# Griffan/FASTQuick

Measured on AMD Instinct MI355X. Metric: paired_150bp_reads_aligned_per_sec, higher is better.
Workload: dtype u32

## Files before the change

fastquick_amd/csrc/fq_align.cpp:

```cpp
#include <algorithm>
#include <atomic>
#include <ctime>
#include <chrono>
#include <climits>
#include <cstdint>
#include <cmath>
#include <cstdio>
#include <cstdlib>
#include <cstring>
#include <memory>
#include <string>
#include <unordered_map>
#include <mutex>
#include <thread>
#include <vector>
#include <pthread.h>
#include <sched.h>

#include "../../include/fastquick_amd.h"
#include "fq_backend.h"
#include "fq_index.h"
#include "fq_pipeline.h"
#include "fq_pool.h"
#include "fq_text_batch.h"
// ... 128 lines not shown
    }
    used = 0; total = 0; last_grow = tl_grow;
  }
  void *alloc(size_t bytes) {
    bytes = (bytes + 63) & ~(size_t)63;
    total += bytes;
    if (blocks.empty() || used + bytes > blocks.back().cap) {
      size_t cap = std::max<size_t>(std::max(bytes, grown(bytes)), (size_t)4 << 20);
      uint8_t *p = (uint8_t *)obtain(cap, true, &cap);
      if (!p) return nullptr;
      blocks.push_back({p, cap});
      used = 0;
    }
    void *r = blocks.back().p + used;
    used += bytes;
    return r;
  }
};

struct FqKnobs {
  uint32_t gap_long_pops = 256;
  int gap_long_always = 0;
  int64_t gap_skip_bound = -1;
  uint32_t gap_long_pops2 = 0;
  int64_t gap_split_hard = 0;
  int64_t gap_pipeline_min = -1;
  int gap_pipeline_segs = 8;
  int64_t gap_nogap_min = 131072;
  uint32_t gap_pool = 2048;
  int gap_no_order = 0;
  int device_turns = 2;
  int device_turn_slots = 1;
  int64_t device_turn_min = 1 << 20;
  int gap_round2_refill = 16;
  int gap_round1_refill = 0;
  int gap_round2_lane_major = 1;
  int gap_round2_waves = 2560;
  int sw_wave_max = 4096;
  int host_threads = -1;
  size_t host_par_min = 32768;
  int64_t md_mask_min = 4096;
  int64_t packed_bulk_min = -1;
  int trace = 0;
};

struct SearchBufs {
  DevBuf<int32_t> work;
  DevBuf<uint32_t> wfull; DevBuf<FqPos> prec; DevBuf<FqGapWork> winfo; DevBuf<uint8_t> bid_end;
  DevBuf<int32_t> order; DevBuf<uint32_t> order_cnt;
  DevBuf<FqAln> aln; DevBuf<uint32_t> naln, status;
  DevBuf<uint32_t> queue, heads; DevBuf<FqEntry> pool;
};

struct fq_ctx {
  FqWorkPool pool;
  const fq_index *ix = nullptr;
  fq_opts_t o{};
  FqKOpts ko{};
  FqKnobs kn;
  fqdev::State *dev = nullptr;
  int max_pairs = 0;
  int debug = 0;
  std::string err;
  fq_serial_hook before_serial = nullptr, after_serial = nullptr;
  void *hook_user = nullptr;
  bool serial_open = false, serial_done = false;
  bool stream_broken = false;
  uint64_t rng = 0;
  fq_isize_t last_ii{};
  std::unordered_map<uint64_t, vector<uint32_t>> kl_cache;
  int g_log_n[256];
  uint8_t maxdiff_lut[FQ_LMAX + 2];
  int n_pairs = 0, stride = 0;
  int in_kind = 0;
  fq_read_batch_t hb{};
  fq_packed_batch_t pb{};
  const fq_text_batch *tb = nullptr;
  PinBuf<uint8_t> p_cseq, p_cqual;
  PinBuf<int32_t> p_clen;
  PinBuf<char> p_cnames;
  DevBuf<char> d_cnames;
  vector<uint16_t> h_len_all;
  int c_stride = 0, c_name_stride = 0;
  DevBuf<uint64_t> d_head[2];
  DevBuf<uint16_t> d_hlen[2];
  DevBuf<uint8_t> d_qlast[2];
  int head_slot = 0;
  const fq_packed_batch_t *pend[2] = {nullptr, nullptr};
  uint64_t pend_serial[2] = {0, 0};
  bool is_pending(int i, const fq_packed_batch_t *b) const { return pend[i] == b && pend_serial[i] == b->serial; }
  DevBuf<uint8_t> d_body, d_pqual;
  DevBuf<uint64_t> d_exc;
  DevBuf<int32_t> d_row_map, d_crow, d_len_c, d_len_all;
  PinBuf<uint8_t> p_body, p_pqual;
  PinBuf<uint64_t> p_exc;
  PinBuf<uint16_t> p_hlen;
  DevBuf<uint16_t> d_blen;
  DevBuf<uint8_t> d_seq, d_qual, d_filtered, d_maxdiff;
  DevBuf<int32_t> d_len, d_len_trim, d_read_list, d_sidx, d_pair_list, d_counts;
  DevBuf<uint64_t> d_counters;
  std::vector<uint64_t> h_counters;
  SearchBufs sb[2];
  DevBuf<uint32_t> d_seg_cnt;
  DevBuf<FqAln> d_hits;
  DevBuf<uint64_t> d_aoff; DevBuf<uint32_t> d_an;
  DevBuf<uint64_t> d_off;
  DevBuf<FqDRec> d_rec, d_grec;
  DevBuf<uint32_t> d_nocc, d_qfirst, d_cnt[3], d_isz;
  DevBuf<uint16_t> d_ntop;
  DevBuf<uint8_t> d_enum, d_cls;
  DevBuf<uint64_t> d_row0, d_scan[3], d_rng, d_grow0;
  DevBuf<int32_t> d_list, d_refmax;
  DevBuf<fq_multi_t> d_multi, d_omulti;
  DevBuf<FqSwTask> d_swslot; DevBuf<FqSwCand> d_swcand;
  DevBuf<FqPairRead> d_greads; DevBuf<FqPairOut> d_gout;
  DevBuf<FqRefTgt> d_reftgt;
  DevBuf<uint16_t> d_cigs, d_ocig;
  DevBuf<fq_isize_t> d_iis;
  DevBuf<fq_result_t> d_orec;
  DevBuf<char> d_omd;
  PinBuf<fq_result_t> p_orec; PinBuf<uint16_t> p_ocig; PinBuf<char> p_omd; PinBuf<fq_multi_t> p_omulti;
  PinBuf<uint16_t> p_ntop; PinBuf<uint32_t> p_isz; PinBuf<int32_t> p_pairs;
  DevBuf<FqAln> d_qaln;
  DevBuf<uint32_t> d_qlen, d_pos, d_qpos, d_qrow, d_qinfo;
  DevBuf<FqPairIsize> d_pisize; DevBuf<int32_t> d_plut, d_glogn; DevBuf<uint64_t> d_pscratch;
  DevBuf<uint64_t> d_qoff;
  DevBuf<FqSwTask> d_swtask;
  DevBuf<FqSwOut> d_swout;
  DevBuf<FqRefTask> d_reftask;
  DevBuf<FqRefOut> d_refout;
  DevBuf<uint16_t> d_cig, d_cigarena;
  DevBuf<uint8_t> d_scratch;
  DevBuf<char> d_md;
  DevBuf<uint16_t> d_mdmask;
  vector<uint8_t> h_filtered;
  vector<int32_t> h_len_trim, h_sub_max;
  const int32_t *h_pair_list = nullptr;
  const FqSurvInfo *h_surv = nullptr;
  Retired retired;
  PinArena arena;
  PinBuf<int32_t> p_i32;
  PinBuf<FqSurvInfo> p_surv;
  PinBuf<uint32_t> p_u32a, p_u32b, p_pos;
  PinBuf<FqAln> p_aln;
  DevBuf<FqSurvInfo> d_surv;
  DevBuf<int32_t> d_sub_max;
  int64_t n_bases_in = 0;
  int emit_flags = 0;
  bool host_rows = true;
  DevBuf<uint8_t> d_equal; PinBuf<uint8_t> p_equal;
  DevBuf<char> d_enames; PinBuf<char> p_enames;
  int e_qstride = 0, e_nstride = 0;
  std::mutex view_mu;
  bool view_ready = false;
  FqSamArgs view{};
  vector<uint8_t> h_eseq;
  DevBuf<uint32_t> d_samlen, d_sammeta; DevBuf<uint64_t> d_samoff; DevBuf<char> d_samtext;
  uint64_t sam_bytes = 0;
  bool sam_ready = false;
  fqdev::State *dev_emit[2] = {nullptr, nullptr};
  PinBuf<char> p_emit[2][2];
  fq_bam *bam = nullptr;
  DevBuf<uint32_t> d_bamlen, d_bammeta, d_zsize; DevBuf<uint64_t> d_bamoff, d_zoff; DevBuf<uint8_t> d_bamrec, d_zstage, d_bamz;
  FqBamCallOut bam_out;
  PinBuf<uint64_t> p_ztotal;
  uint32_t emit_nb = 0;
  std::mutex emit_mu;
  bool emit_pending = false;
  fq_qc *qc = nullptr;
  DevBuf<int32_t> d_qadded;
  DevBuf<uint32_t> d_istlen, d_ptcnt;
  DevBuf<uint64_t> d_istoff, d_ptoff, d_qcnt, d_dupkey;
  DevBuf<char> d_isttext; DevBuf<FqPileEntry> d_pile;
// ... 1721 lines not shown
      c->stats.d2h_bytes += N * sizeof(fq_result_t) + cc * 2 + mm + xx * sizeof(fq_multi_t);
    }
  }
  uint64_t cnt[FQ_C_COUNT];
  c->h_counters.resize((size_t)FQ_C_STRIPES * FQ_C_STRIDE);
  CKS(d2h_staged(c, c->h_counters.data(), c->d_counters.p, c->h_counters.size() * 8));
  CKS(sync_staged(c));
  fold_counters(c->h_counters.data(), cnt);
  CK(fqdev::dzero(c->d_counters.p, c->h_counters.size() * 8));
  if (!N && ((c->emit_flags & FQ_EMIT_SAM) || c->qc || c->bam)) CKS(emit_measure(K));
  if (host_arrays) {
    if (!cc) c->p_ocig.p[0] = 0;
    if (!mm) c->p_omd.p[0] = 0;
    if (!xx) c->p_omulti.p[0] = fq_multi_t{};
  }
  K.trace("result arrays D2H");
  if (cnt[FQ_C_ERR_DRAW0]) {
    c->err = "the drand48 stream drew exactly 0 for the first best hit of a read (once in 2^48 draws): bwa_aln2seq_core then takes no hit and the reference's "
             "record keeps the SA row of the read slot's previous occupant (libbwa/bwase.c:29-41) -- its result is undefined, and so this call is refused";
    return FQ_ELIMIT;
  }
  if (cnt[FQ_C_ERR_CIGAR]) { c->err = "refine: CIGAR longer than the device slot"; return FQ_ELIMIT; }
  if (cnt[FQ_C_ERR_MD]) { c->err = "MD string longer than the device slot"; return FQ_ELIMIT; }
  if (host_arrays) { S.rec = c->p_orec.p; S.cigar = c->p_ocig.p; S.md = c->p_omd.p; S.multi = c->p_omulti.p; }
  else { S.rec = nullptr; S.cigar = nullptr; S.md = nullptr; S.multi = nullptr; }
  S.n_both_unmapped = (int)cnt[FQ_C_UNMAPPED];
  out->n_survivors = n_surv;
  out->n_both_filtered = K.n - n_surv;
  out->n_both_unmapped = S.n_both_unmapped;
  out->pair_idx = S.pair_idx;
  out->rec = S.rec;
  out->cigar = S.cigar;
  out->md = S.md;
  out->multi = S.multi;
  out->isize = K.iis[n_sub - 1];
  out->n_sub = n_sub;
  out->isize_sub = S.isize_sub.data();
  out->n_bases = c->n_bases_in;
  fqdev::time_collect(c->stats.kernel_ms, c->stats.kernel_launches, FQ_K_COUNT);
  c->stats.occ_block_touches += cnt[FQ_C_OCC_WIDTH] + cnt[FQ_C_OCC_GAP] + cnt[FQ_C_OCC_SA];
  c->stats.gap_occ_touches += cnt[FQ_C_OCC_GAP];
  c->stats.width_occ_touches += cnt[FQ_C_OCC_WIDTH];
  c->stats.md_reads += cnt[FQ_C_MD_READS];
  c->stats.host_pairs += (uint64_t)K.n_host_pairs;
  c->stats.gap_nogap_touches += cnt[FQ_C_OCC_NOGAP];
  c->stats.filter_probes += cnt[FQ_C_PROBES];
  c->stats.stack_pops += cnt[FQ_C_POPS];
  c->stats.stack_pushes += cnt[FQ_C_PUSHES];
  if (cnt[FQ_C_MAXPOPS] > c->stats.max_pops_per_read) c->stats.max_pops_per_read = cnt[FQ_C_MAXPOPS];
  c->stats.reads_over_4k_pops += cnt[FQ_C_POPS_GT4K];
  if (cnt[FQ_C_MAXTRIPS] > c->stats.max_wave_trips) c->stats.max_wave_trips = cnt[FQ_C_MAXTRIPS];
  c->stats.wave_trips += cnt[FQ_C_SUMTRIPS];
  c->stats.lane_trips += cnt[FQ_C_LANETRIPS];
  c->stats.sa_rows += cnt[FQ_C_SA_DIRECT];
  c->stats.pairs_on_device += cnt[FQ_C_PAIRS_DEV];
  for (int k = 0; k < 16; ++k) c->stats.dbg[k] += cnt[FQ_C_DBG0 + k];
  c->stats.pairs += K.n;
  c->stats.host_ms_serial += (K.t_serial1 - K.t_host0) - (K.w_serial1 - K.w_host0);
  c->stats.host_ms_pair += (K.t_host1 - K.t_serial1) - (K.w_host1 - K.w_serial1);
  c->stats.host_ms_total += (K.t_host1 - K.t_host0) - (K.w_host1 - K.w_host0);
  c->stats.wall_ms_total += now_ms() - K.t_wall0;
  c->stats.device_wait_ms += c->wait_ms - K.w_call0;
  { timespec ts; clock_gettime(CLOCK_THREAD_CPUTIME_ID, &ts); c->stats.host_cpu_ms += 1e3 * (double)ts.tv_sec + 1e-6 * (double)ts.tv_nsec - K.cpu_call0; }
  K.trace("counters+timers");
  if ((c->emit_flags & FQ_EMIT_SAM) || c->qc || c->bam) CKS(emit_fill(K));
  return FQ_OK;
}
#undef REC

int run_call_stages(fq_ctx *c, fq_result_batch_t *out);
int run_call(fq_ctx *c, fq_result_batch_t *out) {
  c->serial_open = c->serial_done = false;
  const int rc = run_call_stages(c, out);
  if (rc && (c->before_serial || c->after_serial)) {
    c->stream_broken = true;
    if (!c->serial_open && !c->serial_done && c->before_serial) c->before_serial(c->hook_user);
    if (!c->serial_done && c->after_serial) c->after_serial(c->hook_user);
  }
  if (rc) {
    fqdev::copy_discard();
    (void)fqdev::stream_aux(0);
    (void)fqdev::dzero(c->d_counters.p, (size_t)FQ_C_STRIPES * FQ_C_STRIDE * 8);
    (void)fqdev::sync();
    (void)fqdev::copy_wait(0);
    (void)fqdev::copy_wait(1);
  }
  return rc;
}
int run_call_stages(fq_ctx *c, fq_result_batch_t *out) {
  CallInFlight in_flight(c->ix);
  Call K(c);
  K.t_trace = K.t_wall0 = now_ms();
  K.w_call0 = c->wait_ms;
  { timespec ts; clock_gettime(CLOCK_THREAD_CPUTIME_ID, &ts); K.cpu_call0 = 1e3 * (double)ts.tv_sec + 1e-6 * (double)ts.tv_nsec; }
  NodePin pin;
  struct PoolScope { FqWorkPool *prev; explicit PoolScope(FqWorkPool *p) : prev(tl_pool) { tl_pool = p; } ~PoolScope() { tl_pool = prev; } } pool_scope(&c->pool);
  (void)fqdev::stream_aux(0);
  const double grow = c->in_kind == 3 && c->tb && c->n_pairs > 0 && std::min<double>((double)c->max_pairs, (double)c->tb->pairs_behind) > (double)c->n_pairs
                          ? std::min(16.0, std::min<double>((double)c->max_pairs, (double)c->tb->pairs_behind) / (double)c->n_pairs) : 1.0;
  GrowScope grow_scope(grow);
  c->retired.next_call();
  RetiredScope retired_scope(&c->retired);
  if (c->kn.trace) { fprintf(stderr, "[fq]   arena: %zu blocks, last call used %zu bytes:", c->arena.blocks.size(), c->arena.total); for (auto &b : c->arena.blocks) fprintf(stderr, " %zu", b.cap); fprintf(stderr, "\n"); }
  c->arena.reset();
  const fq_opts_t &o = c->o;
  FqBatchState &S = c->st;
  S.clear();
  S.n_pairs = c->n_pairs;
  c->e_qstride = c->e_nstride = 0; c->view_ready = false;
  memset(out, 0, sizeof *out);
  out->n_pairs = c->n_pairs;
  if (c->n_pairs == 0) {
    const int rc0 = emit_measure(K);
    return rc0 ? rc0 : emit_fill(K);
  }
  K.n = c->n_pairs; K.n2 = 2 * K.n; K.B = o.batch_pairs; K.n_sub = (K.n + K.B - 1) / K.B;
  K.par_min = c->kn.host_par_min;
  K.host_threads = call_host_threads(c);
  int rc = c->in_kind == 3 ? stage0_text(K) : c->in_kind == 2 ? stage0_packed(K) : stage0_ascii(K);
  if (rc) return rc;
  S.n_surv = K.n_surv;
  S.batch_pairs = K.B;
  S.sub_lo = K.sub_lo;
  S.pair_idx = c->h_pair_list;
  S.surv = c->h_surv;
  K.trace("stage0 prep+compact");
  if ((rc = stageA_search(K))) return rc;
  K.trace("stageA width+gap");
  if ((rc = stage_records(K))) return rc;
  K.trace("records, SA plan, best-hit counts D2H");
  K.plan.n_chunks = ((size_t)K.n_surv + FQ_RNG_CHUNK_PAIRS - 1) / FQ_RNG_CHUNK_PAIRS;
  K.plan.start = (uint64_t *)c->arena.alloc((K.plan.n_chunks + 1) * 8);
  if (!K.plan.start) { c->err = "out of pinned host memory"; return FQ_ENOMEM; }
  if (!c->before_serial && (size_t)K.n_surv * 2 >= K.par_min) K.plan_thread = std::thread([&K, c] { stageB1_plan(K, c->rng); });
  if ((rc = stage_sa_rows(K))) return rc;
  K.trace("SA enumerate+kernel");
  K.t_host0 = now_ms(); K.w_host0 = c->wait_ms;
  if (c->before_serial) c->before_serial(c->hook_user);
  c->serial_open = true;
  if (c->stream_broken) { c->err = "the stream's state comes from a call that failed (on this rank or on the one before)"; return FQ_EIO; }
  if ((rc = stageB1_main_hit(K))) return rc;
  K.trace("B1 replay + main hit");
  if (o.single_end) K.iis.assign(K.n_sub, fq_isize_t{});
  else {
    stageB2_isize(K);
    c->last_ii = K.iis[K.n_sub - 1];
    if ((rc = stage_kl_cache(K))) return rc;
  }
  K.gate_take(c->qc);
  if (c->after_serial) c->after_serial(c->hook_user);
  c->serial_done = true;
  if (c->stream_broken) { c->err = "the hook that hands the stream's state on failed (fq_ctx_mark_stream_broken)"; return FQ_EIO; }
  K.t_serial1 = now_ms(); K.w_serial1 = c->wait_ms;
  K.trace("B2 isize, (k,l) cache");
  if ((rc = stageB3_pairing(K))) return rc;
  K.trace("B3 pairing+XA");
  if (c->debug && (rc = snapshot_records(K, S.stage_P))) return rc;
  if (!o.single_end && (rc = stageC_mate_sw(K))) return rc;
  K.trace("C mate SW");
  if (c->debug && (rc = snapshot_records(K, S.stage_S))) return rc;
  if ((rc = stageD_refine(K))) return rc;
  K.trace("D refine+MD");
  K.t_host1 = now_ms(); K.w_host1 = c->wait_ms;
  return stage_finish(K, out);
}
}

extern "C" int fq_host_cpus(void) { return (int)effective_cpus(); }
extern "C" int fq_runtime_configure(int hw_queues, int blocking_waits) { return fqdev::runtime_configure(hw_queues, blocking_waits); }
extern "C" int fq_device_count(void) { return fqdev::device_count(); }

extern "C" int fq_align_resident(fq_ctx_t *c, fq_result_batch_t *out) {
  if (!c || !out) return FQ_EINVAL;
  if (c->in_kind != 1) { c->err = "fq_align_resident: no batch uploaded (fq_batch_upload)"; return FQ_EINVAL; }
  if (fqdev::bind(c->dev)) return FQ_ENODEV;
  return run_call(c, out);
}

static int packed_check(fq_ctx_t *c, const fq_packed_batch_t *in) {
  if (!in || in->n_pairs < 0 || (in->n_pairs > 0 && (!in->head || !in->body || in->body_stride < 1 || (in->uniform_len <= 0 && !in->len)))) return FQ_EINVAL;
  if (in->n_exc < 0 || (in->n_exc > 0 && !in->exc)) return FQ_EINVAL;
  if (in->n_pairs > c->max_pairs) { c->err = "batch larger than max_pairs_per_batch"; return FQ_ELIMIT; }
  if (in->uniform_len > 0 && (in->uniform_len < FQ_LMIN || in->uniform_len > FQ_LMAX || (in->uniform_len + 3) / 4 > in->body_stride)) return refuse_length(c);
  if (c->o.trim_qual >= 1 && in->n_pairs > 0 && (!in->qual || in->qual_stride < 1)) { c->err = "quality trimming needs the batch's qualities"; return FQ_EINVAL; }
  if (in->n_pairs > 0 && in->qual_last && !in->qual) { c->err = "qual_last without the quality rows"; return FQ_EINVAL; }
  if ((in->single_end != 0) != (c->o.single_end != 0)) { c->err = c->o.single_end ? "a single-end context takes single-end batches (fq_pack_single_reads_into)" : "a paired-end context takes paired batches"; return FQ_EINVAL; }
  return FQ_OK;
}
extern "C" int fq_packed_prefetch(fq_ctx_t *c, const fq_packed_batch_t *next) {
  if (!c) return FQ_EINVAL;
  int rc = packed_check(c, next);
  if (rc) return rc;
  if (fqdev::bind(c->dev)) return FQ_ENODEV;
  if (next->n_pairs == 0 || c->is_pending(0, next) || c->is_pending(1, next)) return FQ_OK;
  for (int i = 0; i < 2; ++i) if (c->pend[i] == next) c->pend[i] = nullptr;
  const int slot = !c->pend[0] ? 0 : !c->pend[1] ? 1 : -1;
  if (slot < 0) return FQ_OK;
  rc = head_upload(c, next, slot);
  if (rc) return rc;
  c->pend[slot] = next; c->pend_serial[slot] = next->serial;
  return FQ_OK;
}
extern "C" int fq_packed_cancel(fq_ctx_t *c, const fq_packed_batch_t *b) {
  if (!c || !b) return FQ_EINVAL;
  for (int i = 0; i < 2; ++i)
    if (c->pend[i] == b) {
      if (fqdev::bind(c->dev)) return FQ_ENODEV;
      CK(fqdev::copy_wait(i));
      c->pend[i] = nullptr;
    }
  return FQ_OK;
}
extern "C" int fq_align_packed(fq_ctx_t *c, const fq_packed_batch_t *in, fq_result_batch_t *out) {
  if (!c || !out) return FQ_EINVAL;
  int rc = packed_check(c, in);
  if (rc) return broken_stream_call(c, rc);
  if (fqdev::bind(c->dev)) return FQ_ENODEV;
  c->pb = *in;
  c->n_pairs = in->n_pairs;
  c->in_kind = 2;
  if (in->n_pairs > 0) {
    if (c->is_pending(0, in)) { c->head_slot = 0; c->pend[0] = nullptr; }
    else if (c->is_pending(1, in)) { c->head_slot = 1; c->pend[1] = nullptr; }
    else {
      for (int i = 0; i < 2; ++i) if (c->pend[i] == in) c->pend[i] = nullptr;
      c->head_slot = !c->pend[0] ? 0 : 1;
      c->pend[c->head_slot] = nullptr;
      rc = head_upload(c, in, c->head_slot);
      if (rc) return broken_stream_call(c, rc);
    }
  }
  return run_call(c, out);
}

extern "C" int fq_stream_run(fq_ctx_t *const *ctxs, int32_t n_streams, const fq_packed_batch_t *const *const *batches, const int32_t *n_batches, const int32_t *first,
                             int32_t n_calls, int32_t flags, fq_stream_call_fn on_call, void *user, int64_t *survivors_out) {
  if (!ctxs || n_streams < 1 || !batches || !n_batches || n_calls < 0) return FQ_EINVAL;
  for (int s = 0; s < n_streams; ++s) if (!ctxs[s] || !batches[s] || n_batches[s] < 1) return FQ_EINVAL;
  for (int s = 0; s < n_streams; ++s) for (int t = 0; t < s; ++t) if (ctxs[s] == ctxs[t]) return FQ_EINVAL;
  std::vector<int> rcs((size_t)n_streams, FQ_OK);
  std::vector<int64_t> surv((size_t)n_streams, 0);
  static const bool trace_cpu = [] { const char *e = getenv("FASTQUICK_TRACE"); return e && *e && *e != '0'; }();
  std::vector<double> cpu_pre((size_t)n_streams, 0.0), cpu_call((size_t)n_streams, 0.0);
  auto thread_cpu_ms = [] { timespec ts; clock_gettime(CLOCK_THREAD_CPUTIME_ID, &ts); return 1e3 * (double)ts.tv_sec + 1e-6 * (double)ts.tv_nsec; };
  auto run = [&](int s) {
    fq_ctx_t *c = ctxs[s];
    const int nb = n_batches[s];
    int cur = (first ? first[s] : 0) % nb;
    if (cur < 0) cur += nb;
    fq_result_batch_t res;
    for (int k = 0; k < n_calls; ++k) {
      const int nxt = (cur + 1) % nb;
      int rc = FQ_OK;
      const bool pre = nxt != cur && (k + 1 < n_calls || (flags & FQ_STREAM_PREFETCH_BEYOND));
      const double c0 = trace_cpu ? thread_cpu_ms() : 0.0;
      if (pre) rc = fq_packed_prefetch(c, batches[s][nxt]);
      const double c1 = trace_cpu ? thread_cpu_ms() : 0.0;
      if (!rc) rc = fq_align_packed(c, batches[s][cur], &res);
      if (trace_cpu) { cpu_pre[(size_t)s] += c1 - c0; cpu_call[(size_t)s] += thread_cpu_ms() - c1; }
      if (!rc) { surv[(size_t)s] += res.n_survivors; if (on_call) rc = on_call(user, s, k, &res); }
      if (rc) { rcs[(size_t)s] = rc; if (pre) (void)fq_packed_cancel(c, batches[s][nxt]); return; }
      cur = nxt;
    }
  };
  std::vector<std::thread> th;
  for (int s = 1; s < n_streams; ++s) th.emplace_back(run, s);
  run(0);
  for (auto &t : th) t.join();
  if (survivors_out) for (int s = 0; s < n_streams; ++s) survivors_out[s] = surv[(size_t)s];
  if (trace_cpu && n_calls > 0) {
    double a = 0, b = 0;
    for (int s = 0; s < n_streams; ++s) { a += cpu_pre[(size_t)s]; b += cpu_call[(size_t)s]; }
    fprintf(stderr, "TRACE - fq_stream_run: %d streams x %d calls; CPU time of a stream's thread per call: prefetch %.3f ms, call %.3f ms\n", n_streams, n_calls,
            a / ((double)n_streams * n_calls), b / ((double)n_streams * n_calls));
  }
  for (int rc : rcs) if (rc) return rc;
  return FQ_OK;
}

extern "C" int fq_align_text(fq_ctx_t *c, const fq_text_batch *tb, fq_result_batch_t *out) {
  if (!c || !out || !tb) return FQ_EINVAL;
  int rc = FQ_OK;
  if (tb->n_pairs < 0 || (tb->n_pairs > 0 && (!tb->d_head || !tb->d_rec || !tb->d_text[0] || !tb->d_names))) rc = FQ_EINVAL;
  else if (tb->n_pairs > c->max_pairs) { c->err = "batch larger than max_pairs_per_batch"; rc = FQ_ELIMIT; }
  else if ((tb->single_end != 0) != (c->o.single_end != 0)) { c->err = "single-end / paired-end batch on a context of the other kind"; rc = FQ_EINVAL; }
  else if (tb->device != c->ix->device) { c->err = "the batch lives on another device than the context's index"; rc = FQ_EINVAL; }
  else if (tb->uniform_len > 0 && (tb->uniform_len < FQ_LMIN || tb->uniform_len > FQ_LMAX)) rc = refuse_length(c);
  if (rc) return broken_stream_call(c, rc);
  if (fqdev::bind(c->dev)) return FQ_ENODEV;
  c->tb = tb;
  c->n_pairs = tb->n_pairs;
  c->in_kind = 3;
  return run_call(c, out);
}

static const uint64_t kStateGood = 0x31545351465full, kStateBroken = 0x58545351465full;
extern "C" int64_t fq_ctx_state_export(const fq_ctx_t *c, void *buf, int64_t cap) {
  if (!c) return FQ_EINVAL;
  int64_t need = 8 + 8 + (int64_t)sizeof(fq_isize_t) + 8;
  for (const auto &kv : c->kl_cache) need += 16 + 4 * (int64_t)kv.second.size();
  if (!buf || cap < need) return need;
  uint8_t *p = (uint8_t *)buf;
  const uint64_t mark = c->stream_broken ? kStateBroken : kStateGood;
  memcpy(p, &mark, 8); p += 8;
  memcpy(p, &c->rng, 8); p += 8;
  memcpy(p, &c->last_ii, sizeof(fq_isize_t)); p += sizeof(fq_isize_t);
  const uint64_t n = c->kl_cache.size();
  memcpy(p, &n, 8); p += 8;
  for (const auto &kv : c->kl_cache) {
    const uint64_t m = kv.second.size();
    memcpy(p, &kv.first, 8); p += 8;
    memcpy(p, &m, 8); p += 8;
    memcpy(p, kv.second.data(), 4 * m); p += 4 * m;
  }
  return need;
}
extern "C" int fq_ctx_state_move(fq_ctx_t *to, fq_ctx_t *from) {
  if (!to || !from || to == from) return FQ_EINVAL;
  if (from->stream_broken) { to->stream_broken = true; to->err = "the stream's state comes from a call that failed"; return FQ_EIO; }
  to->rng = from->rng; to->last_ii = from->last_ii;
  to->kl_cache.swap(from->kl_cache);
  from->kl_cache.clear();
  return FQ_OK;
}
extern "C" int fq_ctx_state_import(fq_ctx_t *c, const void *buf, int64_t len) {
  if (!c || !buf || len < (int64_t)(24 + sizeof(fq_isize_t))) return FQ_EINVAL;
  const uint8_t *p = (const uint8_t *)buf, *end = p + len;
  uint64_t mark;
  memcpy(&mark, p, 8); p += 8;
  if (mark == kStateBroken) { c->stream_broken = true; c->err = "the stream's state comes from a call that failed on another rank"; return FQ_EIO; }
  if (mark != kStateGood) return FQ_EINVAL;
  uint64_t rng, n;
  fq_isize_t ii;
  memcpy(&rng, p, 8); p += 8;
  memcpy(&ii, p, sizeof(fq_isize_t)); p += sizeof(fq_isize_t);
  memcpy(&n, p, 8); p += 8;
  std::unordered_map<uint64_t, vector<uint32_t>> cache;
  bool ok = n <= (uint64_t)(end - p) / 16;
  for (uint64_t i = 0; ok && i < n; ++i) {
    if (end - p < 16) { ok = false; break; }
    uint64_t key, m;
    memcpy(&key, p, 8); p += 8;
    memcpy(&m, p, 8); p += 8;
    if (m > (uint64_t)(end - p) / 4) { ok = false; break; }
// ... 152 lines not shown
```

fastquick_amd/csrc/fq_backend.h:

```cpp
#pragma once
#include "fq_kernels.h"
#include "fq_records.h"
#include "fq_frontend.h"
#include "fq_emit.h"
#include "fq_deflate.h"

namespace fqdev {

struct State;
struct Tune {
  int gap_coop_waves = 0;
  int gap_waves_per_cu = 0, gap_refill_min = 0, gap_order_asc = 0, filter_no_turns = 0, refine_lanes = 0;
  int spin_sync = 0;
  int gap_generic_opts = 0;
  int width_both_strands = 0;
  int prep_priority = 0;
  int sw_serial_reverse = 0;
};
int runtime_configure(int hw_queues, int blocking_waits);
int device_count();
State *state_create(int device_ordinal);
void state_destroy(State *s);
int bind(State *s);
Tune *tune(State *s);
const char *last_error();
bool is_real_gpu();
void device_turn_begin(int slots = 1);
void device_turn_end();

void *dmalloc(size_t bytes);
void dfree(void *p);
void *hmalloc(size_t bytes);
void hfree(void *p);
int h2d(void *dst, const void *src, size_t bytes);
int d2h(void *dst, const void *src, size_t bytes);
int copy_pinned(void *dst, const void *src, size_t bytes, int to_device);
int d2d(void *dst, const void *src, size_t bytes);
int dzero(void *dst, size_t bytes);
int dfill(void *dst, int byte, size_t bytes);
int sync();
int h2d_copy(void *dst, const void *src, size_t bytes);
int copy_record(int slot);
int copy_wait(int slot);
void copy_discard();
int compute_wait_copy(int slot);
int copy_flush_now();

void time_begin(int kid);
void time_end(int kid);
void time_collect(double ms[], uint64_t launches[], int n_ids);
inline thread_local uint64_t dp_launches[FQ_DP_COUNT] = {};

int launch_prep(const FqPrepArgs &a);
int launch_compact(const uint8_t *filtered, int n_pairs, int32_t *read_list, int32_t *sidx, int32_t *pair_list, int32_t *counts);
int launch_surv_gather(const int32_t *pair_list, int n_surv, int n_pairs, const int32_t *len_trim, const uint8_t *filtered, const int32_t *sidx, FqSurvInfo *out);
int launch_prep_packed(const FqPrepPackedArgs &a);
int launch_surv_map(const int32_t *pair_list, int n_surv, int n_pairs, const uint8_t *filtered, const int32_t *sidx, FqSurvInfo *out,
                    int32_t *row_map, int32_t *read_list_c, int32_t *crow_of);
int launch_unpack(const FqUnpackArgs &a);
int launch_patch(const FqPatchArgs &a);
int launch_trim(const FqTrimArgs &a);
int launch_trim_all(const FqTrimAllArgs &a);
int launch_width(const FqWidthArgs &a);
int launch_order(const uint8_t *bid_end, int n, int n_hard, int32_t *order, uint32_t *cnt);
int gap_lane_slots(const FqGapArgs &a);
int launch_gap(const FqGapArgs &a);
int launch_scan(const uint32_t *in, uint64_t *out, uint32_t n);
int launch_pack_aln(const FqAln *aln, const uint32_t *n_aln, const uint64_t *off, uint32_t cap, uint32_t n_work, FqAln *packed);
int launch_sa(const FqSaArgs &a);
int stream_aux(int on);
int stream_fork();
int stream_join();
int stream_mark(int k);
int stream_wait_mark(int k);
int launch_collect(const int32_t *order, const uint32_t *split, int n_work, int seg, int n_seg, const uint32_t *status, const int32_t *work, int32_t *out, uint32_t *count);
int launch_rec(int op, const FqRecArgs &a, int64_t n);
int launch_aln_index(const int32_t *work, const uint32_t *status, const uint64_t *off, const uint32_t *naln, uint64_t base, uint64_t *aoff, uint32_t *an, int n);
int launch_sam(int op, const FqSamArgs &a, int64_t n);
int launch_bam(int op, const FqBamArgs &a, int64_t n);
int launch_deflate(const FqDeflateArgs &a);
int launch_deflate_pack(const FqDeflatePackArgs &a);
int launch_qc(int op, const FqQcArgs &a, int64_t n);
int launch_dup_rehash(const uint64_t *old, uint64_t old_cap, uint64_t *tab, uint64_t mask);
int launch_sw(const FqSwArgs &a);
int launch_sw_serial(const FqSwArgs &a);
int launch_refine(const FqRefineArgs &a);

const FqzCrcConst *crc_const();
int launch_inflate(const FqInflateArgs &a);
int launch_inflate2(const FqInflateArgs &a, const FqInflateArgs &b);
int launch_nl_index(const uint8_t *text, uint32_t n, uint32_t lo, uint32_t *nl, uint32_t cap, uint32_t *count);
int launch_tok_rec(const FqTokArgs &a);
int launch_tok_pieces(const FqTokArgs &a);
int launch_slot_bases(const FqSlotArgs &a);
int launch_slot_names(const FqSlotArgs &a);
int launch_text_gather(const FqTextGatherArgs &a);
int launch_text_trim_all(const FqTextTrimArgs &a);
int dfill32(void *dst, uint32_t v, size_t n_words);

}
```

fastquick_amd/csrc/fq_device.hip:

```cpp
#include <hip/hip_runtime.h>
#include <hip/hip_ext.h>

#include <algorithm>
#include <condition_variable>
#include <atomic>
#include <cstdio>
#include <cstdlib>
#include <cstring>
#include <mutex>
#include <string>
#include <unordered_map>
#include <vector>
#include <sys/mman.h>
#include <sys/syscall.h>
#include <unistd.h>

#include "fq_backend.h"

namespace fqdev {

struct Pending { int kid; hipEvent_t a, b; };
struct State {
  int device = 0;
  hipStream_t stream = nullptr;
  hipStream_t main_stream = nullptr, aux_stream = nullptr;
  hipEvent_t fork_ev = nullptr, join_ev = nullptr;
  hipEvent_t marks[4] = {nullptr, nullptr, nullptr, nullptr};
  hipEvent_t prio_fork = nullptr;
  hipStream_t copy_stream = nullptr;
  hipEvent_t copy_done[2] = {nullptr, nullptr};
  hipEvent_t prep_done = nullptr;
  hipEvent_t sync_ev = nullptr;
  std::vector<Pending> pending;
  std::vector<hipEvent_t> free_events;
  hipEvent_t open_begin[16] = {};
  struct SmallCopy { uint8_t *dst; const uint8_t *src; size_t bytes; };
  SmallCopy small[8];
  int n_small = 0;
  uint64_t *scan_tmp = nullptr; size_t scan_tmp_n = 0;
  uint32_t *cmp_cnt = nullptr; uint64_t *cmp_off = nullptr; size_t cmp_n = 0;
  Tune tune;
};
static thread_local State *g_cur = nullptr;
static thread_local std::string g_err;
#define g_stream (g_cur->stream)

#define FQ_HIP(call)                                                                         \
  do {                                                                                       \
    hipError_t e_ = (call);                                                                  \
    if (e_ != hipSuccess) {                                                                  \
      g_err = std::string(#call) + ": " + hipGetErrorString(e_);                             \
      return -3;                                                                             \
    }                                                                                        \
  } while (0)

int copy_flush();
#define FQ_PRE() do { if (copy_flush()) return -3; } while (0)
void copy_discard() { if (g_cur) g_cur->n_small = 0; }
int copy_flush_now() { FQ_PRE(); return 0; }

const char *last_error() { return g_err.c_str(); }
bool is_real_gpu() { return true; }

static int set_kernel_attributes();
static std::mutex g_dev_mu;
static bool g_dev_ready[64];
static hipEvent_t g_prep_last[64];
static State *g_prep_owner[64];
static hipStream_t g_copy_streams[64][2];
static unsigned g_copy_next[64];
static std::mutex g_turn_mu[64];
static std::condition_variable g_turn_cv[64];
static int g_turn_held[64];
static int g_ctx_count[64];
static hipStream_t g_prio_stream[64];
static bool g_queue_warned = false;
static int g_rt_blocking_waits = 0;
int runtime_configure(int hw_queues, int blocking_waits) {
  if (hw_queues > 0) {
    char b[16];
    snprintf(b, sizeof b, "%d", hw_queues);
    setenv("GPU_MAX_HW_QUEUES", b, 0);
  }
  g_rt_blocking_waits = blocking_waits ? 1 : 0;
  return 0;
}

int device_count() { int n = 0; if (hipGetDeviceCount(&n) != hipSuccess) { (void)hipGetLastError(); return 0; } return n < 0 ? 0 : n; }
void device_turn_begin(int slots) {
  const int d = g_cur->device;
  std::unique_lock<std::mutex> lk(g_turn_mu[d]);
  g_turn_cv[d].wait(lk, [&] { return g_turn_held[d] < (slots < 1 ? 1 : slots); });
  ++g_turn_held[d];
}
void device_turn_end() {
  const int d = g_cur->device;
  { std::lock_guard<std::mutex> lk(g_turn_mu[d]); --g_turn_held[d]; }
  g_turn_cv[d].notify_all();
}

State *state_create(int dev) {
  int n = 0;
  if (hipGetDeviceCount(&n) != hipSuccess || n <= 0) { g_err = "no HIP device visible"; return nullptr; }
  if (dev < 0 || dev >= n || dev >= 64) { g_err = "device ordinal out of range"; return nullptr; }
  if (hipSetDevice(dev) != hipSuccess) { g_err = "hipSetDevice failed"; return nullptr; }
  g_cur = nullptr;
  {
    std::lock_guard<std::mutex> lk(g_dev_mu);
    if (!g_dev_ready[dev]) {
      if (g_rt_blocking_waits) { (void)hipSetDeviceFlags(hipDeviceScheduleBlockingSync); (void)hipGetLastError(); }
      if (set_kernel_attributes()) return nullptr;
      g_dev_ready[dev] = true;
    }
    const char *q = getenv("GPU_MAX_HW_QUEUES");
    const int queues = q && atoi(q) > 0 ? atoi(q) : 4;
    if (++g_ctx_count[dev] + 2 > queues && !g_queue_warned) {
      g_queue_warned = true;
      fprintf(stderr, "fastquick_amd: %d alignment contexts on device %d with GPU_MAX_HW_QUEUES=%d: contexts will share hardware queues and wait for each other's kernels "
                      "(fq_runtime_configure(contexts + 4, ..) or GPU_MAX_HW_QUEUES before the process makes its first HIP call)\n", g_ctx_count[dev], dev, queues);
    }
  }
  State *s = new State;
  s->device = dev;
  bool ok = hipStreamCreateWithFlags(&s->stream, hipStreamNonBlocking) == hipSuccess &&
            hipEventCreateWithFlags(&s->copy_done[0], hipEventDisableTiming | hipEventBlockingSync) == hipSuccess &&
            hipEventCreateWithFlags(&s->copy_done[1], hipEventDisableTiming | hipEventBlockingSync) == hipSuccess &&
            hipEventCreateWithFlags(&s->prep_done, hipEventDisableTiming) == hipSuccess &&
            hipEventCreateWithFlags(&s->sync_ev, hipEventDisableTiming | hipEventBlockingSync) == hipSuccess;
  if (!ok) { g_err = "stream / event creation failed"; state_destroy(s); return nullptr; }
  s->main_stream = s->stream;
  return s;
}
void state_destroy(State *s) {
  if (!s) return;
  (void)hipSetDevice(s->device);
  g_cur = nullptr;
  s->stream = s->main_stream ? s->main_stream : s->stream;
  if (s->aux_stream) { (void)hipStreamSynchronize(s->aux_stream); (void)hipStreamDestroy(s->aux_stream); }
  if (s->sync_ev) (void)hipEventDestroy(s->sync_ev);
  if (s->fork_ev) (void)hipEventDestroy(s->fork_ev);
  if (s->join_ev) (void)hipEventDestroy(s->join_ev);
  for (hipEvent_t m : s->marks) if (m) (void)hipEventDestroy(m);
  if (s->prio_fork) (void)hipEventDestroy(s->prio_fork);
  if (s->stream) (void)hipStreamSynchronize(s->stream);
  if (s->copy_stream) (void)hipStreamSynchronize(s->copy_stream);
  {
    std::lock_guard<std::mutex> lk(g_dev_mu);
    if (g_prep_owner[s->device] == s) { g_prep_owner[s->device] = nullptr; g_prep_last[s->device] = nullptr; }
    if (g_ctx_count[s->device] > 0) --g_ctx_count[s->device];
  }
  for (auto &p : s->pending) { (void)hipEventDestroy(p.a); (void)hipEventDestroy(p.b); }
  for (auto e : s->free_events) (void)hipEventDestroy(e);
  for (auto e : s->copy_done) if (e) (void)hipEventDestroy(e);
  if (s->prep_done) (void)hipEventDestroy(s->prep_done);
  if (s->scan_tmp) (void)hipFree(s->scan_tmp);
  if (s->cmp_cnt) (void)hipFree(s->cmp_cnt);
  if (s->cmp_off) (void)hipFree(s->cmp_off);
  if (s->stream) (void)hipStreamDestroy(s->stream);
  delete s;
}
Tune *tune(State *s) { return &s->tune; }
int bind(State *s) {
  if (!s) { g_err = "no device state"; return -3; }
  if (g_cur != s) { FQ_HIP(hipSetDevice(s->device)); g_cur = s; }
  return 0;
}

void *dmalloc(size_t bytes) {
  void *p = nullptr;
  if (hipMalloc(&p, bytes ? bytes : 16) != hipSuccess) { g_err = "hipMalloc failed (" + std::to_string(bytes) + " B)"; return nullptr; }
  return p;
}
void dfree(void *p) { if (p) (void)hipFree(p); }
static const size_t kRegisterMin = (size_t)4 << 20;
static std::mutex g_reg_mu;
static std::unordered_map<void *, size_t> g_registered;
static int device_numa_node(int dev) {
  static std::mutex mu;
  static std::unordered_map<int, int> cache;
  std::lock_guard<std::mutex> lk(mu);
  auto it = cache.find(dev);
  if (it != cache.end()) return it->second;
  int node = -1;
  char bus[64] = {0};
  if (hipDeviceGetPCIBusId(bus, (int)sizeof bus, dev) == hipSuccess) {
    for (char *c = bus; *c; ++c) if (*c >= 'A' && *c <= 'F') *c = (char)(*c - 'A' + 'a');
    const std::string path = std::string("/sys/bus/pci/devices/") + bus + "/numa_node";
    if (FILE *f = fopen(path.c_str(), "r")) { if (fscanf(f, "%d", &node) != 1) node = -1; fclose(f); }
  } else (void)hipGetLastError();
  cache[dev] = node;
  return node;
}
static void prefer_node(void *m, size_t len, int node) {
  if (node < 0 || node >= 1024) return;
  unsigned long mask[16] = {0};
  mask[node / (8 * sizeof(unsigned long))] |= 1ul << (node % (8 * sizeof(unsigned long)));
  (void)syscall(SYS_mbind, m, len, 1 , mask, (unsigned long)(8 * sizeof mask + 1), 0u);
}
void *hmalloc(size_t bytes) {
  static const bool use_register = [] { const char *e = getenv("FASTQUICK_PIN_REGISTER"); return !(e && *e == '0'); }();
  if (use_register && bytes >= kRegisterMin) {
    const size_t len = (bytes + ((size_t)2 << 20) - 1) & ~(((size_t)2 << 20) - 1);
    void *m = mmap(nullptr, len, PROT_READ | PROT_WRITE, MAP_PRIVATE | MAP_ANONYMOUS, -1, 0);
    if (m != MAP_FAILED) {
      (void)madvise(m, len, MADV_HUGEPAGE);
      int dev = 0;
      if (hipGetDevice(&dev) == hipSuccess) prefer_node(m, len, device_numa_node(dev)); else (void)hipGetLastError();
      if (hipHostRegister(m, len, hipHostRegisterDefault) == hipSuccess) {
        std::lock_guard<std::mutex> lk(g_reg_mu);
        g_registered[m] = len;
        return m;
      }
      (void)hipGetLastError();
      munmap(m, len);
    }
  }
  void *p = nullptr;
  if (hipHostMalloc(&p, bytes ? bytes : 16, hipHostMallocDefault) != hipSuccess) { g_err = "hipHostMalloc failed"; return nullptr; }
  return p;
}
void hfree(void *p) {
  if (!p) return;
  size_t len = 0;
  {
    std::lock_guard<std::mutex> lk(g_reg_mu);
    auto it = g_registered.find(p);
    if (it != g_registered.end()) { len = it->second; g_registered.erase(it); }
  }
  if (len) { (void)hipHostUnregister(p); munmap(p, len); }
  else (void)hipHostFree(p);
}
int h2d(void *dst, const void *src, size_t bytes) { FQ_PRE(); if (bytes) FQ_HIP(hipMemcpyAsync(dst, src, bytes, hipMemcpyHostToDevice, g_stream)); return 0; }
int d2h(void *dst, const void *src, size_t bytes) { FQ_PRE(); if (bytes) FQ_HIP(hipMemcpyAsync(dst, src, bytes, hipMemcpyDeviceToHost, g_stream)); return 0; }
int d2d(void *dst, const void *src, size_t bytes) { FQ_PRE(); if (bytes) FQ_HIP(hipMemcpyAsync(dst, src, bytes, hipMemcpyDeviceToDevice, g_stream)); return 0; }
int dzero(void *dst, size_t bytes) { FQ_PRE(); if (bytes) FQ_HIP(hipMemsetAsync(dst, 0, bytes, g_stream)); return 0; }
int dfill(void *dst, int byte, size_t bytes) { FQ_PRE(); if (bytes) FQ_HIP(hipMemsetAsync(dst, byte, bytes, g_stream)); return 0; }
int sync() {
  FQ_PRE();
  if (g_cur->tune.spin_sync || !g_cur->sync_ev) { FQ_HIP(hipStreamSynchronize(g_stream)); return 0; }
  FQ_HIP(hipEventRecord(g_cur->sync_ev, g_stream));
  FQ_HIP(hipEventSynchronize(g_cur->sync_ev));
  return 0;
}
int stream_aux(int on) {
  FQ_PRE();
  if (on && !g_cur->aux_stream) {
    FQ_HIP(hipStreamCreateWithFlags(&g_cur->aux_stream, hipStreamNonBlocking));
    FQ_HIP(hipEventCreateWithFlags(&g_cur->fork_ev, hipEventDisableTiming));
    FQ_HIP(hipEventCreateWithFlags(&g_cur->join_ev, hipEventDisableTiming));
  }
  g_cur->stream = on ? g_cur->aux_stream : g_cur->main_stream;
  return 0;
}
int stream_fork() {
  FQ_PRE();
  if (!g_cur->aux_stream) return 0;
  FQ_HIP(hipEventRecord(g_cur->fork_ev, g_cur->main_stream));
  FQ_HIP(hipStreamWaitEvent(g_cur->aux_stream, g_cur->fork_ev, 0));
  return 0;
}
int stream_join() {
  FQ_PRE();
  if (!g_cur->aux_stream) return 0;
  FQ_HIP(hipEventRecord(g_cur->join_ev, g_cur->aux_stream));
  FQ_HIP(hipStreamWaitEvent(g_cur->main_stream, g_cur->join_ev, 0));
  return 0;
}
int stream_mark(int k) {
  FQ_PRE();
  hipEvent_t &m = g_cur->marks[k & 3];
  if (!m) FQ_HIP(hipEventCreateWithFlags(&m, hipEventDisableTiming));
  FQ_HIP(hipEventRecord(m, g_stream));
  return 0;
}
int stream_wait_mark(int k) {
  FQ_PRE();
  hipEvent_t m = g_cur->marks[k & 3];
  if (m) FQ_HIP(hipStreamWaitEvent(g_stream, m, 0));
  return 0;
}
static int copy_stream_get() {
  if (g_cur->copy_stream) return 0;
  std::lock_guard<std::mutex> lk(g_dev_mu);
  const int dev = g_cur->device;
  for (int k = 0; k < 2; ++k)
    if (!g_copy_streams[dev][k]) FQ_HIP(hipStreamCreateWithFlags(&g_copy_streams[dev][k], hipStreamNonBlocking));
  g_cur->copy_stream = g_copy_streams[dev][g_copy_next[dev]++ & 1];
  return 0;
}
int h2d_copy(void *dst, const void *src, size_t bytes) {
  if (copy_stream_get()) return -3;
  if (bytes) FQ_HIP(hipMemcpyAsync(dst, src, bytes, hipMemcpyHostToDevice, g_cur->copy_stream));
  return 0;
}
int copy_record(int slot) { if (copy_stream_get()) return -3; FQ_HIP(hipEventRecord(g_cur->copy_done[slot & 1], g_cur->copy_stream)); return 0; }
int copy_wait(int slot) { FQ_HIP(hipEventSynchronize(g_cur->copy_done[slot & 1])); return 0; }
int compute_wait_copy(int slot) { FQ_PRE(); FQ_HIP(hipStreamWaitEvent(g_stream, g_cur->copy_done[slot & 1], 0)); return 0; }

struct FqCopySet { uint8_t *dst[8]; const uint8_t *src[8]; size_t bytes[8]; };
__global__ void __launch_bounds__(256) k_copy_bytes(FqCopySet cs) {
  uint8_t *dst = cs.dst[blockIdx.y];
  const uint8_t *src = cs.src[blockIdx.y];
  const size_t bytes = cs.bytes[blockIdx.y];
  const size_t n16 = ((((uintptr_t)dst | (uintptr_t)src) & 15) == 0) ? bytes / 16 : 0;
  const size_t t = (size_t)blockIdx.x * blockDim.x + threadIdx.x, stride = (size_t)gridDim.x * blockDim.x;
  for (size_t i = t; i < n16; i += stride) ((uint4 *)dst)[i] = ((const uint4 *)src)[i];
  for (size_t i = n16 * 16 + t; i < bytes; i += stride) dst[i] = src[i];
}
static const size_t kSmallCopy = (size_t)8 << 20;
int copy_flush() {
  State *s = g_cur;
  if (!s || s->n_small == 0) return 0;
  FqCopySet cs;
  size_t most = 0;
  for (int k = 0; k < 8; ++k) {
    const bool on = k < s->n_small;
    cs.dst[k] = on ? s->small[k].dst : nullptr; cs.src[k] = on ? s->small[k].src : nullptr; cs.bytes[k] = on ? s->small[k].bytes : 0;
    if (on) most = std::max(most, s->small[k].bytes);
  }
  const int n = s->n_small;
  s->n_small = 0;
  const unsigned blocks = (unsigned)std::min<size_t>(256, (most / 16 + 255) / 256 + 1);
  hipLaunchKernelGGL(k_copy_bytes, dim3(blocks, (unsigned)n), dim3(256), 0, s->stream, cs);
  FQ_HIP(hipGetLastError());
  return 0;
}
int copy_pinned(void *dst, const void *src, size_t bytes, int to_device) {
  if (!bytes) return 0;
  if (bytes > kSmallCopy) { FQ_PRE(); FQ_HIP(hipMemcpyAsync(dst, src, bytes, to_device ? hipMemcpyHostToDevice : hipMemcpyDeviceToHost, g_stream)); return 0; }
  if (g_cur->n_small == 8) FQ_PRE();
  g_cur->small[g_cur->n_small++] = {(uint8_t *)dst, (const uint8_t *)src, bytes};
  return 0;
}

static hipEvent_t get_event() {
  if (!g_cur->free_events.empty()) { hipEvent_t e = g_cur->free_events.back(); g_cur->free_events.pop_back(); return e; }
  hipEvent_t e;
  (void)hipEventCreate(&e);
  return e;
}
void time_begin(int kid) { (void)copy_flush(); hipEvent_t e = get_event(); (void)hipEventRecord(e, g_stream); g_cur->open_begin[kid] = e; }
void time_end(int kid) { (void)copy_flush(); hipEvent_t e = get_event(); (void)hipEventRecord(e, g_stream); g_cur->pending.push_back({kid, g_cur->open_begin[kid], e}); }
static void kernel_events(int kid, hipEvent_t *a, hipEvent_t *b) { *a = get_event(); *b = get_event(); g_cur->pending.push_back({kid, *a, *b}); }
void time_collect(double ms[], uint64_t launches[], int n_ids) {
  std::vector<decltype(g_cur->pending)::value_type> later;
  for (auto &p : g_cur->pending) {
    if (hipEventQuery(p.b) == hipErrorNotReady) { later.push_back(p); continue; }
    float t = 0.f;
    if (hipEventElapsedTime(&t, p.a, p.b) == hipSuccess && p.kid < n_ids) { ms[p.kid] += t; launches[p.kid] += 1; }
    g_cur->free_events.push_back(p.a);
    g_cur->free_events.push_back(p.b);
  }
  g_cur->pending.swap(later);
}

static inline unsigned nblk(uint64_t n, unsigned b) { return (unsigned)((n + b - 1) / b); }

__global__ void __launch_bounds__(256) k_prep(FqPrepArgs a) {
  const int r = blockIdx.x * blockDim.x + threadIdx.x;
  if (r < a.n_reads) fq_prep_thread(a, r);
}
extern __shared__ __align__(16) unsigned char fq_dyn_lds[];
__global__ void __launch_bounds__(256) k_width(FqWidthArgs a) {
  uint8_t *seed_bits = (uint8_t *)fq_dyn_lds;
  const int w = blockIdx.x * blockDim.x + threadIdx.x;
  if (w < a.n_work) fq_width_read(a, w, seed_bits + threadIdx.x, 256);
}
__global__ void __launch_bounds__(256) k_width_strand(FqWidthArgs a) {
  uint8_t *seed_bits = (uint8_t *)fq_dyn_lds;
  const int xcd = blockIdx.x & 7, strand = xcd >> 2;
  const int q = (int)(blockIdx.x >> 3) * 4 + (xcd & 3);
  const int w = q * 256 + threadIdx.x;
  if (w < a.n_work) fq_width_strand(a, w, strand, seed_bits + threadIdx.x, 256);
}
struct FqQueueFetch {
  uint32_t *cursor;
  int n_work;
  __device__ uint32_t operator()(uint32_t n) const { return atomicAdd(cursor, n); }
};
#if defined(FQ_GAP_WPE)
// ... 1195 lines not shown
```

Measured before the change: 761.2 million.

## Triple-buffer packed head uploads and prefetch two batches ahead in stream run

```diff
diff --git a/fastquick_amd/csrc/fq_align.cpp b/fastquick_amd/csrc/fq_align.cpp
--- a/fastquick_amd/csrc/fq_align.cpp
+++ b/fastquick_amd/csrc/fq_align.cpp
@@ -234,13 +234,16 @@
   DevBuf<char> d_cnames;
   vector<uint16_t> h_len_all;
   int c_stride = 0, c_name_stride = 0;
-  DevBuf<uint64_t> d_head[2];
-  DevBuf<uint16_t> d_hlen[2];
-  DevBuf<uint8_t> d_qlast[2];
+  DevBuf<uint64_t> d_head[FQ_HEAD_SLOTS];
+  DevBuf<uint16_t> d_hlen[FQ_HEAD_SLOTS];
+  DevBuf<uint8_t> d_qlast[FQ_HEAD_SLOTS];
   int head_slot = 0;
-  const fq_packed_batch_t *pend[2] = {nullptr, nullptr};
-  uint64_t pend_serial[2] = {0, 0};
+  const fq_packed_batch_t *pend[FQ_HEAD_SLOTS] = {};
+  uint64_t pend_serial[FQ_HEAD_SLOTS] = {};
   bool is_pending(int i, const fq_packed_batch_t *b) const { return pend[i] == b && pend_serial[i] == b->serial; }
+  int pending_slot(const fq_packed_batch_t *b) const { for (int i = 0; i < FQ_HEAD_SLOTS; ++i) if (is_pending(i, b)) return i; return -1; }
+  int free_slot() const { for (int i = 0; i < FQ_HEAD_SLOTS; ++i) if (!pend[i]) return i; return -1; }
+  void forget(const fq_packed_batch_t *b) { for (auto &q : pend) if (q == b) q = nullptr; }
   DevBuf<uint8_t> d_body, d_pqual;
   DevBuf<uint64_t> d_exc;
   DevBuf<int32_t> d_row_map, d_crow, d_len_c, d_len_all;
@@ -2128,8 +2131,7 @@
     (void)fqdev::stream_aux(0);
     (void)fqdev::dzero(c->d_counters.p, (size_t)FQ_C_STRIPES * FQ_C_STRIDE * 8);
     (void)fqdev::sync();
-    (void)fqdev::copy_wait(0);
-    (void)fqdev::copy_wait(1);
+    for (int i = 0; i < FQ_HEAD_SLOTS; ++i) (void)fqdev::copy_wait(i);
   }
   return rc;
 }
@@ -2238,9 +2240,9 @@
   int rc = packed_check(c, next);
   if (rc) return rc;
   if (fqdev::bind(c->dev)) return FQ_ENODEV;
-  if (next->n_pairs == 0 || c->is_pending(0, next) || c->is_pending(1, next)) return FQ_OK;
-  for (int i = 0; i < 2; ++i) if (c->pend[i] == next) c->pend[i] = nullptr;
-  const int slot = !c->pend[0] ? 0 : !c->pend[1] ? 1 : -1;
+  if (next->n_pairs == 0 || c->pending_slot(next) >= 0) return FQ_OK;
+  c->forget(next);
+  const int slot = c->free_slot();
   if (slot < 0) return FQ_OK;
   rc = head_upload(c, next, slot);
   if (rc) return rc;
@@ -2249,7 +2251,7 @@
 }
 extern "C" int fq_packed_cancel(fq_ctx_t *c, const fq_packed_batch_t *b) {
   if (!c || !b) return FQ_EINVAL;
-  for (int i = 0; i < 2; ++i)
+  for (int i = 0; i < FQ_HEAD_SLOTS; ++i)
     if (c->pend[i] == b) {
       if (fqdev::bind(c->dev)) return FQ_ENODEV;
       CK(fqdev::copy_wait(i));
@@ -2266,11 +2268,12 @@
   c->n_pairs = in->n_pairs;
   c->in_kind = 2;
   if (in->n_pairs > 0) {
-    if (c->is_pending(0, in)) { c->head_slot = 0; c->pend[0] = nullptr; }
-    else if (c->is_pending(1, in)) { c->head_slot = 1; c->pend[1] = nullptr; }
+    const int held = c->pending_slot(in);
+    if (held >= 0) { c->head_slot = held; c->pend[held] = nullptr; }
     else {
-      for (int i = 0; i < 2; ++i) if (c->pend[i] == in) c->pend[i] = nullptr;
-      c->head_slot = !c->pend[0] ? 0 : 1;
+      c->forget(in);
+      const int slot = c->free_slot();
+      c->head_slot = slot >= 0 ? slot : FQ_HEAD_SLOTS - 1;
       c->pend[c->head_slot] = nullptr;
       rc = head_upload(c, in, c->head_slot);
       if (rc) return broken_stream_call(c, rc);
@@ -2297,15 +2300,21 @@
     fq_result_batch_t res;
     for (int k = 0; k < n_calls; ++k) {
       const int nxt = (cur + 1) % nb;
-      int rc = FQ_OK;
-      const bool pre = nxt != cur && (k + 1 < n_calls || (flags & FQ_STREAM_PREFETCH_BEYOND));
+      const fq_packed_batch_t *now = batches[s][cur];
+      const fq_packed_batch_t *ahead[2] = {batches[s][nxt], batches[s][(cur + 2) % nb]};
+      for (int a = 0; a < 2; ++a)
+        if (ahead[a] == now || (a && ahead[a] == ahead[0]) || !(k + 1 + a < n_calls || (flags & FQ_STREAM_PREFETCH_BEYOND))) ahead[a] = nullptr;
       const double c0 = trace_cpu ? thread_cpu_ms() : 0.0;
-      if (pre) rc = fq_packed_prefetch(c, batches[s][nxt]);
+      for (const fq_packed_batch_t *b : ahead) if (b) (void)fq_packed_prefetch(c, b);
       const double c1 = trace_cpu ? thread_cpu_ms() : 0.0;
-      if (!rc) rc = fq_align_packed(c, batches[s][cur], &res);
+      int rc = fq_align_packed(c, now, &res);
       if (trace_cpu) { cpu_pre[(size_t)s] += c1 - c0; cpu_call[(size_t)s] += thread_cpu_ms() - c1; }
       if (!rc) { surv[(size_t)s] += res.n_survivors; if (on_call) rc = on_call(user, s, k, &res); }
-      if (rc) { rcs[(size_t)s] = rc; if (pre) (void)fq_packed_cancel(c, batches[s][nxt]); return; }
+      if (rc) {
+        rcs[(size_t)s] = rc;
+        for (int a = 1; a <= 2; ++a) (void)fq_packed_cancel(c, batches[s][(cur + a) % nb]);
+        return;
+      }
       cur = nxt;
     }
   };
diff --git a/fastquick_amd/csrc/fq_backend.h b/fastquick_amd/csrc/fq_backend.h
--- a/fastquick_amd/csrc/fq_backend.h
+++ b/fastquick_amd/csrc/fq_backend.h
@@ -39,6 +39,7 @@
 int dzero(void *dst, size_t bytes);
 int dfill(void *dst, int byte, size_t bytes);
 int sync();
+#define FQ_HEAD_SLOTS 3
 int h2d_copy(void *dst, const void *src, size_t bytes);
 int copy_record(int slot);
 int copy_wait(int slot);
diff --git a/fastquick_amd/csrc/fq_device.hip b/fastquick_amd/csrc/fq_device.hip
--- a/fastquick_amd/csrc/fq_device.hip
+++ b/fastquick_amd/csrc/fq_device.hip
@@ -28,7 +28,7 @@
   hipEvent_t marks[4] = {nullptr, nullptr, nullptr, nullptr};
   hipEvent_t prio_fork = nullptr;
   hipStream_t copy_stream = nullptr;
-  hipEvent_t copy_done[2] = {nullptr, nullptr};
+  hipEvent_t copy_done[FQ_HEAD_SLOTS] = {};
   hipEvent_t prep_done = nullptr;
   hipEvent_t sync_ev = nullptr;
   std::vector<Pending> pending;
@@ -123,10 +123,9 @@
   State *s = new State;
   s->device = dev;
   bool ok = hipStreamCreateWithFlags(&s->stream, hipStreamNonBlocking) == hipSuccess &&
-            hipEventCreateWithFlags(&s->copy_done[0], hipEventDisableTiming | hipEventBlockingSync) == hipSuccess &&
-            hipEventCreateWithFlags(&s->copy_done[1], hipEventDisableTiming | hipEventBlockingSync) == hipSuccess &&
             hipEventCreateWithFlags(&s->prep_done, hipEventDisableTiming) == hipSuccess &&
             hipEventCreateWithFlags(&s->sync_ev, hipEventDisableTiming | hipEventBlockingSync) == hipSuccess;
+  for (hipEvent_t &e : s->copy_done) ok = ok && hipEventCreateWithFlags(&e, hipEventDisableTiming | hipEventBlockingSync) == hipSuccess;
   if (!ok) { g_err = "stream / event creation failed"; state_destroy(s); return nullptr; }
   s->main_stream = s->stream;
   return s;
@@ -288,14 +287,15 @@
   g_cur->copy_stream = g_copy_streams[dev][g_copy_next[dev]++ & 1];
   return 0;
 }
+static inline int head_slot(int slot) { return (int)((unsigned)slot % FQ_HEAD_SLOTS); }
 int h2d_copy(void *dst, const void *src, size_t bytes) {
   if (copy_stream_get()) return -3;
   if (bytes) FQ_HIP(hipMemcpyAsync(dst, src, bytes, hipMemcpyHostToDevice, g_cur->copy_stream));
   return 0;
 }
-int copy_record(int slot) { if (copy_stream_get()) return -3; FQ_HIP(hipEventRecord(g_cur->copy_done[slot & 1], g_cur->copy_stream)); return 0; }
-int copy_wait(int slot) { FQ_HIP(hipEventSynchronize(g_cur->copy_done[slot & 1])); return 0; }
-int compute_wait_copy(int slot) { FQ_PRE(); FQ_HIP(hipStreamWaitEvent(g_stream, g_cur->copy_done[slot & 1], 0)); return 0; }
+int copy_record(int slot) { if (copy_stream_get()) return -3; FQ_HIP(hipEventRecord(g_cur->copy_done[head_slot(slot)], g_cur->copy_stream)); return 0; }
+int copy_wait(int slot) { FQ_HIP(hipEventSynchronize(g_cur->copy_done[head_slot(slot)])); return 0; }
+int compute_wait_copy(int slot) { FQ_PRE(); FQ_HIP(hipStreamWaitEvent(g_stream, g_cur->copy_done[head_slot(slot)], 0)); return 0; }
 
 struct FqCopySet { uint8_t *dst[8]; const uint8_t *src[8]; size_t bytes[8]; };
 __global__ void __launch_bounds__(256) k_copy_bytes(FqCopySet cs) {
```

Result: no change. 768.9 million, median of 4 (+1.0%).
